# sourmash-bio/sourmash

Measured on AMD Instinct MI355X. Metric: Gbase/s sketched (k=31, scaled=1000), higher is better.
Workload: dtype u64; 1 GPU; C2: sketch synthetic random DNA resident in HBM as ASCII, per GPU 1000 records of 10000000 bases (10000000000 bases, 10000001000 bytes with their separators), k=31 scaled=1000 seed=42; one step = k-mer kernel + radix sort + unique; records_per_gpu=1000, record_len=10000000, bases_per_gpu=10000000000, bytes_per_gpu=10000001000, ksize=31, scaled=1000, unique_hashes_rank0=9998668, unique_hashes_job=9998668, collectives=none (the exchange runs with --full)

## Files before the change

include/sourmash_amd.h:

```cpp
#ifndef SOURMASH_AMD_H_INCLUDED
#define SOURMASH_AMD_H_INCLUDED

#include <stdarg.h>
#include <stdbool.h>
#include <stdint.h>
#include <stdlib.h>

#ifdef __cplusplus
extern "C" {
#endif


enum {
  HASH_FUNCTIONS_MURMUR64_DNA = 1,
  HASH_FUNCTIONS_MURMUR64_PROTEIN = 2,
  HASH_FUNCTIONS_MURMUR64_DAYHOFF = 3,
  HASH_FUNCTIONS_MURMUR64_HP = 4,
};
typedef uint32_t HashFunctions;

enum {
  SOURMASH_ERROR_CODE_NO_ERROR = 0,
  SOURMASH_ERROR_CODE_PANIC = 1,
  SOURMASH_ERROR_CODE_INTERNAL = 2,
// ... 166 lines not shown
SourmashHyperLogLog *hll_with_error_rate(double error_rate, uintptr_t ksize);

bool nodegraph_count(SourmashNodegraph *ptr, uint64_t h);
bool nodegraph_count_kmer(SourmashNodegraph *ptr, const char *kmer);
double nodegraph_expected_collisions(const SourmashNodegraph *ptr);
void nodegraph_free(SourmashNodegraph *ptr);
SourmashNodegraph *nodegraph_from_buffer(const char *ptr, uintptr_t insize);
SourmashNodegraph *nodegraph_from_path(const char *filename);
uintptr_t nodegraph_get(const SourmashNodegraph *ptr, uint64_t h);
uintptr_t nodegraph_get_kmer(const SourmashNodegraph *ptr, const char *kmer);
const uint64_t *nodegraph_hashsizes(const SourmashNodegraph *ptr, uintptr_t *size);
uintptr_t nodegraph_ksize(const SourmashNodegraph *ptr);
uintptr_t nodegraph_matches(const SourmashNodegraph *ptr, const SourmashKmerMinHash *mh_ptr);
SourmashNodegraph *nodegraph_new(void);
uintptr_t nodegraph_noccupied(const SourmashNodegraph *ptr);
uintptr_t nodegraph_ntables(const SourmashNodegraph *ptr);
void nodegraph_save(const SourmashNodegraph *ptr, const char *filename);
const uint8_t *nodegraph_to_buffer(const SourmashNodegraph *ptr, uint8_t compression, uintptr_t *size);
void nodegraph_update(SourmashNodegraph *ptr, const SourmashNodegraph *optr);
void nodegraph_update_mh(SourmashNodegraph *ptr, const SourmashKmerMinHash *optr);
SourmashNodegraph *nodegraph_with_tables(uintptr_t ksize, uintptr_t starting_size, uintptr_t n_tables);


int32_t smgpu_device_count(void);
bool smgpu_available(void);

void smgpu_minhash_add_buffer(SourmashKmerMinHash *ptr, const char *buf, uintptr_t len, bool force);

uint32_t smgpu_minhash_add_sequence_rc(SourmashKmerMinHash *ptr, const char *sequence, uintptr_t len, bool force);
void smgpu_minhash_flush(SourmashKmerMinHash *ptr);
uint64_t smgpu_minhash_pending_bytes(const SourmashKmerMinHash *ptr);
uint64_t smgpu_signature_add_file(SourmashSignature *ptr, const char *path, uint64_t *n_records);
SourmashSignature **smgpu_sketch_files(const char *const *paths, uintptr_t n, const SourmashComputeParameters *params,
                                       uint32_t n_threads, uint64_t *total_bases);
uint64_t smgpu_minhash_add_file(SourmashKmerMinHash *ptr, const char *path, uint64_t *n_records);
uint64_t smgpu_gunzip_files(const char *const *paths, uintptr_t n, uint8_t *out, uint64_t capacity, uint64_t *lens, double *stats);
void smgpu_sigload_counters(uint64_t *out);
void smgpu_gunzip_counters(uint64_t *out);

uint64_t smgpu_sketch_workspace_bytes(uint64_t out_capacity);
uint64_t smgpu_sketch_dna_raw(const uint8_t *d_seq, uint64_t len, uint32_t ksize, uint64_t seed, uint64_t max_hash,
                              uint64_t *d_out, uint64_t out_capacity, uint64_t *d_result, void *d_workspace,
                              uint64_t workspace_bytes, void *stream);
uint64_t smgpu_sketch_records_workspace_bytes(uint64_t pair_capacity, uint64_t n_records);
uint64_t smgpu_sketch_records_raw(const uint8_t *d_seq, uint64_t len, const uint64_t *d_starts, uint64_t n_records,
                                  uint32_t ksize, uint64_t seed, uint64_t max_hash, uint64_t *d_hashes, uint64_t *d_abunds,
                                  uint64_t capacity, uint64_t *d_offsets, uint64_t *d_result, void *d_workspace,
                                  uint64_t workspace_bytes, void *stream);
void smgpu_sketch_records_kernel_raw(const uint8_t *d_seq, uint64_t len, uint32_t ksize, uint64_t seed, uint64_t max_hash,
                                     uint64_t *d_hashes, uint64_t *d_positions, uint64_t capacity, uint64_t *d_count, void *stream);
SourmashSignature **smgpu_sketch_file_singleton(const char *path, const SourmashComputeParameters *params, uintptr_t *n);
void smgpu_sketch_dna_kernel_raw(const uint8_t *d_seq, uint64_t len, uint32_t ksize, uint64_t seed, uint64_t max_hash,
                                 uint64_t *d_out, uint64_t out_capacity, uint64_t *d_count, void *stream);
uint64_t smgpu_sort_unique_raw(uint64_t *d_keys, uint64_t n, uint64_t *d_out, uint64_t *d_n_out, void *d_workspace,
                               uint64_t workspace_bytes, void *stream);
uint64_t smgpu_sketch_residues_kernels_raw(const uint8_t *d_seq, uint64_t len, uint32_t k_aa, uint32_t hash_function, uint64_t seed,
                                           uint64_t max_hash, bool translate, uint8_t *d_aa, uint64_t aa_capacity, uint64_t *d_out,
                                           uint64_t out_capacity, uint64_t *d_count, void *stream);
void smgpu_synth_dna_raw(uint8_t *d_out, uint64_t start, uint64_t n, uint64_t seed, uint64_t record_len, void *stream);

void smgpu_compare_raw(const uint64_t *d_hashes, const uint64_t *d_offsets, uint32_t n, uint32_t row_lo,
                       uint32_t row_hi, uint32_t *d_common, double *d_jaccard, void *stream);
void smgpu_compare_blocks_raw(const uint64_t *d_hashes, const uint64_t *d_offsets, uint32_t n, uint32_t rb_first,
                              uint32_t rb_stride, uint32_t rb_count, uint32_t *d_common, void *stream);
void smgpu_symmetrize_raw(uint32_t *d_common, uint32_t n, void *stream);
void smgpu_jaccard_raw(const uint32_t *d_common, const uint64_t *d_offsets, uint32_t n, uint32_t row_lo,
                       uint32_t row_hi, double *d_jaccard, void *stream);
typedef struct SmgpuBitIndex SmgpuBitIndex;
SmgpuBitIndex *smgpu_bitindex_new(const uint64_t *d_hashes, const uint64_t *d_offsets, uint32_t n, void *stream);
SmgpuBitIndex *smgpu_bitindex_new_ex(const uint64_t *d_hashes, const uint64_t *d_offsets, uint32_t n, uint64_t total_hashes,
                                     uint32_t threshold, bool one_shot, void *stream);
void smgpu_bitindex_free(SmgpuBitIndex *ptr);
uint64_t smgpu_bitindex_universe(const SmgpuBitIndex *ptr);
uint32_t smgpu_bitindex_builder(const SmgpuBitIndex *ptr);
void smgpu_bitindex_stats(const SmgpuBitIndex *ptr, uint64_t *frequent_hashes, uint64_t *rare_pairs, uint32_t *threshold);
void smgpu_bitindex_compare_raw(const SmgpuBitIndex *ptr, uint32_t rb_first, uint32_t rb_stride, uint32_t rb_count,
                                uint32_t *d_common, void *stream);
void smgpu_bitindex_compare_upper_raw(const SmgpuBitIndex *ptr, uint32_t rb_first, uint32_t rb_stride, uint32_t rb_count,
                                      uint32_t *d_common, void *stream);
void smgpu_host_pow_f64(const double *x, const double *y, uintptr_t ny, double *out, uintptr_t n, uint32_t n_threads);
uintptr_t smgpu_first_invalid_dna_byte(const char *seq, uintptr_t len);
void smgpu_compare_all_pairs(const SourmashKmerMinHash *const *mhs, uintptr_t n, uint32_t *common_out,
                             double *jaccard_out);
void smgpu_compare_all_pairs_mixed(const SourmashKmerMinHash *const *mhs, uintptr_t n, const uint32_t *class_of,
                                   const uint64_t *class_max_hash, uintptr_t n_classes, uint32_t *common_out, uint64_t *sizes_out);
void smgpu_signatures_sketch_views(const SourmashSignature *const *sigs, uintptr_t n, const SourmashKmerMinHash **out_mhs,
                                   uint64_t *params);
void smgpu_minhashes_params(const SourmashKmerMinHash *const *mhs, uintptr_t n, uint64_t *params);
void *smgpu_host_alloc(uintptr_t bytes);
void smgpu_host_free(void *ptr);
void smgpu_xfer_stats(uint64_t *out5, bool reset);
void smgpu_xfer_roundtrip(const void *const *pieces, const uint64_t *lens, uintptr_t n, void *out, uint64_t out_bytes);
void smgpu_compare_num_all_pairs(const SourmashKmerMinHash *const *mhs, uintptr_t n, uint32_t *common_out, uint32_t *union_out,
                                 double *jaccard_out);
void smgpu_compare_angular_all_pairs(const SourmashKmerMinHash *const *mhs, uintptr_t n, double *sims_out, uint64_t *prod_out,
                                     uint64_t *sumsq_out);
void smgpu_host_angular_f64(const uint64_t *prod, const uint64_t *sumsq, uintptr_t n, double *out, uint32_t n_threads);
void smgpu_compare_num_raw(const uint64_t *d_hashes, const uint64_t *d_offsets, const uint32_t *d_nums, uint32_t n,
                           uint32_t *d_common, uint32_t *d_union, double *d_jaccard, void *stream);
void smgpu_compare_abund_raw(const uint64_t *d_hashes, const uint64_t *d_abunds, const uint64_t *d_offsets, uint32_t n, bool narrow,
                             uint32_t *d_common, uint64_t *d_prod, uint64_t *d_sumsq, void *stream);
void smgpu_compare_abund_raw_n(const uint64_t *d_hashes, const uint64_t *d_abunds, const uint64_t *d_offsets, uint32_t n,
                               uint64_t total_hashes, bool narrow, uint32_t *d_common, uint64_t *d_prod, uint64_t *d_sumsq, void *stream);

typedef struct SmgpuSketchSet SmgpuSketchSet;
typedef struct SmgpuCounter SmgpuCounter;
// ... 106 lines not shown
```

sourmash_amd/csrc/capi.cpp:

```cpp
#if defined(__SSE2__)
#include <emmintrin.h>
#endif
#include <hip/hip_runtime_api.h>
#include <stdio.h>
#include <string.h>
#include <chrono>
#include <cmath>
#include <fstream>
#include <memory>
#include <sstream>
#include <thread>
#include "../../include/sourmash_amd.h"
#include "collection.hpp"
#include <fcntl.h>
#include <sys/mman.h>
#include <sys/stat.h>
#include <unistd.h>
#include "device_ctx.hpp"
#include "hostxfer.hpp"
#include "pargz.hpp"
#include "ingest.hpp"
#include "sigload.hpp"
#include "murmur3.hpp"
#include "residues.hpp"
// ... 773 lines not shown
    return (uint64_t)out_capacity * 8 + sort_unique_temp_bytes(out_capacity) + 512;
}

uint64_t smgpu_sketch_dna_raw(const uint8_t* d_seq, uint64_t len, uint32_t ksize, uint64_t seed, uint64_t max_hash,
                              uint64_t* d_out, uint64_t cap, uint64_t* d_result, void* d_ws, uint64_t ws_bytes,
                              void* stream) {
    uint64_t ret = ~0ull;
    landing_void([&] {
        hipStream_t st = (hipStream_t)stream;
        if (ws_bytes < smgpu_sketch_workspace_bytes(cap)) throw err_internal("workspace too small (smgpu_sketch_workspace_bytes)");
        uint64_t* d_raw = (uint64_t*)d_ws;
        void* d_tmp = (char*)d_ws + ((cap * 8 + 255) / 256) * 256;
        const size_t tmp_bytes = (size_t)(ws_bytes - ((cap * 8 + 255) / 256) * 256);
        const uint64_t thr = max_hash ? max_hash : ~0ull;
        check_dna_ksize(ksize);
        hip_check(hipMemsetAsync(d_result, 0, 16, st), "memset");
        hip_check(sketch_dna_launch(d_seq, len, ksize, seed, thr, d_raw, (unsigned long long*)d_result, cap, st), "sketch_dna");
        unsigned long long kept = 0;
        hip_check(hipMemcpyAsync(&kept, d_result, 8, hipMemcpyDeviceToHost, st), "D2H");
        hip_check(hipStreamSynchronize(st), "sync");
        if (kept > cap)
            throw err_internal("output capacity too small: " + std::to_string(kept) + " kept hashes > capacity " + std::to_string(cap));
        int bits = 64;
        if (thr != ~0ull) { bits = 1; while (bits < 64 && (thr >> bits)) ++bits; }
        hip_check(sort_unique(d_raw, kept, d_out, nullptr, d_result + 1, d_tmp, tmp_bytes, bits, st), "sort_unique");
        unsigned long long nu = 0;
        hip_check(hipMemcpyAsync(&nu, d_result + 1, 8, hipMemcpyDeviceToHost, st), "D2H");
        hip_check(hipStreamSynchronize(st), "sync");
        ret = nu;
    });
    return ret;
}

uint64_t smgpu_sort_unique_raw(uint64_t* d_keys, uint64_t n, uint64_t* d_out, uint64_t* d_n_out, void* d_ws, uint64_t ws_bytes, void* stream) {
    uint64_t ret = ~0ull;
    landing_void([&] {
        hipStream_t st = (hipStream_t)stream;
        if (ws_bytes < sort_unique_temp_bytes(n)) throw err_internal("workspace too small (smgpu_sketch_workspace_bytes)");
        hip_check(sort_unique(d_keys, n, d_out, nullptr, d_n_out, d_ws, (size_t)ws_bytes, 64, st), "sort_unique");
        unsigned long long nu = 0;
        hip_check(hipMemcpyAsync(&nu, d_n_out, 8, hipMemcpyDeviceToHost, st), "D2H");
        hip_check(hipStreamSynchronize(st), "sync");
        ret = nu;
    });
    return ret;
}

void smgpu_sketch_dna_kernel_raw(const uint8_t* d_seq, uint64_t len, uint32_t ksize, uint64_t seed, uint64_t max_hash,
                                 uint64_t* d_out, uint64_t cap, uint64_t* d_count, void* stream) {
    landing_void([&] {
        check_dna_ksize(ksize);
        hip_check(sketch_dna_launch(d_seq, len, ksize, seed, max_hash ? max_hash : ~0ull, d_out,
                                    (unsigned long long*)d_count, cap, (hipStream_t)stream), "sketch_dna");
    });
}

uint64_t smgpu_sketch_residues_kernels_raw(const uint8_t* d_seq, uint64_t len, uint32_t k_aa, uint32_t hash_function, uint64_t seed,
                                           uint64_t max_hash, bool translate, uint8_t* d_aa, uint64_t aa_capacity, uint64_t* d_out,
                                           uint64_t cap, uint64_t* d_count, void* stream) {
    return landing<uint64_t>([&]() -> uint64_t {
        if (hash_function < HF_PROTEIN || hash_function > HF_HP) throw err_internal("hash_function must be protein, dayhoff or hp");
        const uint64_t n_aa = translate ? translated_bytes(len) : len;
        if (((n_aa + 7) & ~7ull) > aa_capacity) throw err_internal("d_aa is too small: " + std::to_string(n_aa) + " residues need " + std::to_string((n_aa + 7) & ~7ull) + " bytes");
        hipStream_t st = (hipStream_t)stream;
        if (translate) hip_check(translate_launch(d_seq, len, hash_function, d_aa, st), "translate");
        else hip_check(residues_launch(d_seq, len, hash_function, d_aa, st), "residues");
        hip_check(residue_windows_launch(d_aa, translate && len < 3 ? 0 : n_aa, k_aa, seed, max_hash ? max_hash : ~0ull, d_out, (unsigned long long*)d_count, cap,
                                         false, st), "residue windows");
        return n_aa;
    });
}

void smgpu_synth_dna_raw(uint8_t* d_out, uint64_t start, uint64_t n, uint64_t seed, uint64_t record_len, void* stream) {
    landing_void([&] { hip_check(synth_dna_launch(d_out, start, n, seed, record_len, (hipStream_t)stream), "synth_dna"); });
}

void smgpu_compare_raw(const uint64_t* d_hashes, const uint64_t* d_offsets, uint32_t n, uint32_t row_lo, uint32_t row_hi,
                       uint32_t* d_common, double* d_jaccard, void* stream) {
    landing_void([&] {
        if (!d_common) throw err_internal("d_common is required");
        hip_check(compare_counts_launch(d_hashes, d_offsets, n, row_lo, row_hi, d_common, (hipStream_t)stream), "compare");
        if (d_jaccard)
            hip_check(jaccard_from_counts_launch(d_common, d_offsets, n, row_lo, row_hi, d_jaccard, (hipStream_t)stream), "jaccard");
    });
}

void smgpu_compare_blocks_raw(const uint64_t* d_hashes, const uint64_t* d_offsets, uint32_t n, uint32_t rb_first,
                              uint32_t rb_stride, uint32_t rb_count, uint32_t* d_common, void* stream) {
    landing_void([&] {
        hip_check(compare_blocks_launch(d_hashes, d_offsets, n, rb_first, rb_stride, rb_count, d_common, (hipStream_t)stream),
                  "compare_blocks");
    });
}
void smgpu_symmetrize_raw(uint32_t* d_common, uint32_t n, void* stream) {
    landing_void([&] { hip_check(symmetrize_launch(d_common, n, (hipStream_t)stream), "symmetrize"); });
}
void smgpu_jaccard_raw(const uint32_t* d_common, const uint64_t* d_offsets, uint32_t n, uint32_t row_lo, uint32_t row_hi,
                       double* d_jaccard, void* stream) {
    landing_void([&] {
        hip_check(jaccard_from_counts_launch(d_common, d_offsets, n, row_lo, row_hi, d_jaccard, (hipStream_t)stream), "jaccard");
    });
}

struct BitIndex {
    uint32_t n = 0, words_per_row = 0;
    uint64_t universe = 0, total = 0;
// ... 2124 lines not shown
```

sourmash_amd/csrc/device_api.hpp:

```cpp
#pragma once
#include <hip/hip_runtime.h>
#include <stdint.h>
#include <stddef.h>

namespace smg {

hipError_t sketch_dna_launch(const uint8_t* d_seq, uint64_t len, uint32_t k, uint64_t seed, uint64_t thr,
                             uint64_t* d_out, unsigned long long* d_count, uint64_t cap, hipStream_t stream);
struct SketchMultiOut { uint64_t thr; uint64_t* out; unsigned long long* count; uint64_t cap; };
bool sketch_dna_multi_supported(const uint32_t* ks, int n);
hipError_t sketch_dna_multi_launch(const uint8_t* d_new, uint64_t n_new, const uint32_t* ks, int n, uint64_t seed, const SketchMultiOut* outs,
                                   hipStream_t stream);
hipError_t sketch_dna_words_launch(const uint8_t* d_seq, uint64_t len, uint32_t k, uint64_t seed, uint64_t thr, uint64_t* d_out,
                                   unsigned long long* d_count, uint64_t cap, bool dense, hipStream_t stream);
uint32_t sketch_dna_max_k();
hipError_t kmer_hashes_launch(const uint8_t* d_seq, uint64_t len, uint32_t k, uint64_t seed, uint64_t* d_out,
                              uint64_t n_kmers, hipStream_t stream);
hipError_t first_invalid_launch(const uint8_t* d_seq, uint64_t len, unsigned long long* d_first, hipStream_t stream);

hipError_t hll_dna_launch(const uint8_t* d_seq, uint64_t len, uint32_t k, uint32_t p, uint32_t* d_regs, hipStream_t stream);
hipError_t hll_hashes_launch(const uint64_t* d_hashes, uint64_t n, uint32_t p, uint32_t* d_regs, bool skip_zero, hipStream_t stream);
hipError_t hll_pack_launch(const uint32_t* d_regs, uint32_t n, uint8_t* d_out, hipStream_t stream);

struct NgTable { uint64_t size, magic, off; };
struct NgDev {
    const NgTable* tabs = nullptr;
    uint32_t n_tables = 0;
    uint32_t* words = nullptr;
    uint64_t n_words = 0;
    uint64_t t0_words = 0;
    unsigned long long* occ = nullptr;
};
hipError_t nodegraph_dna_launch(const uint8_t* d_seq, uint64_t len, uint32_t k, const NgDev& g, hipStream_t stream);
hipError_t nodegraph_hashes_launch(const uint64_t* d_hashes, uint64_t n, const NgDev& g, hipStream_t stream);
hipError_t nodegraph_matches_launch(const uint64_t* d_hashes, const uint64_t* d_offsets, uint64_t n_rows, const NgDev& g,
                                    uint64_t* d_out, hipStream_t stream);

hipError_t residues_launch(const uint8_t* d_seq, uint64_t len, uint32_t hash_function, uint8_t* d_aa, hipStream_t stream);
uint64_t translated_bytes(uint64_t len);
hipError_t translate_launch(const uint8_t* d_seq, uint64_t len, uint32_t hash_function, uint8_t* d_aa, hipStream_t stream);
hipError_t residue_windows_launch(const uint8_t* d_aa, uint64_t n, uint32_t k, uint64_t seed, uint64_t thr, uint64_t* d_out,
                                  unsigned long long* d_count, uint64_t cap, bool dense, hipStream_t stream);

size_t sort_unique_temp_bytes(uint64_t n);
struct TagSegment { uint64_t src, dst, n; };
hipError_t tag_gather_launch(const uint64_t* d_src, const TagSegment* d_segs, uint32_t n_segs, uint64_t* d_dst, int hbits, hipStream_t stream);
hipError_t sort_unique(uint64_t* d_keys, uint64_t n, uint64_t* d_out, uint64_t* d_counts, uint64_t* d_n_out,
                       void* d_temp, size_t temp_bytes, int bits, hipStream_t stream);

size_t sort_pairs_temp_bytes(uint64_t n);
hipError_t sort_pairs(const uint64_t* d_keys_in, uint64_t* d_keys_out, const uint64_t* d_vals_in, uint64_t* d_vals_out, uint64_t n,
                      int bits, void* d_temp, size_t temp_bytes, hipStream_t stream);
size_t rle_pairs_temp_bytes(uint64_t n);
hipError_t rle_pairs(const uint64_t* d_a, const uint64_t* d_b, uint64_t n, uint64_t* d_out_a, uint64_t* d_out_b, uint64_t* d_counts,
                     uint64_t* d_n_out, void* d_temp, size_t temp_bytes, hipStream_t stream);

hipError_t records_pairs_launch(const uint8_t* d_seq, uint64_t len, uint32_t k, uint64_t seed, uint64_t thr, uint64_t* d_hash,
                                uint64_t* d_pos, unsigned long long* d_count, uint64_t cap, hipStream_t stream);
hipError_t records_check_starts_launch(const uint64_t* d_starts, uint64_t n_records, uint64_t len, unsigned long long* d_bad,
                                       hipStream_t stream);
size_t records_csr_temp_bytes(uint64_t n_pairs);
// ... 58 lines not shown
```

sourmash_amd/csrc/kmer_core.hpp:

```cpp
#pragma once
#include "murmur3.hpp"
#include <utility>

namespace smg {

SMG_HD uint32_t perm_b32(uint32_t hi, uint32_t lo, uint32_t sel) {
#if defined(__HIP_DEVICE_COMPILE__)
    return __builtin_amdgcn_perm(hi, lo, sel);
#else
    const uint64_t v = ((uint64_t)hi << 32) | lo;
    uint32_t r = 0;
    for (int i = 0; i < 4; ++i) {
        const uint32_t s = (sel >> (8 * i)) & 0xff;
        uint32_t b;
        if (s < 8) b = (uint32_t)(v >> (8 * s)) & 0xff;
        else if (s == 0x0c) b = 0;
        else b = 0xff;
        r |= b << (8 * i);
    }
    return r;
#endif
}

SMG_HD uint32_t alignbyte_b32(uint32_t hi, uint32_t lo, uint32_t n) {
// ... 188 lines not shown
        }
    }
    static_assert(G::NBYTES <= 192 && K <= 128 && P <= 64, "window too long for the 192-bit validity mask");
    (
        [&] {
            const Mmh3Open open = PosOps<K, P, O>::template hash_open<PLAIN>(U, C, seed);
            if constexpr (EARLY) {
                if (!any_lane(early_may_keep(open, lim))) return;
            }
            const uint64_t h = mmh3_close<PLAIN>(open);
            bool ok = (h - 1) < thr;
            if (anybad != 0) {
                uint64_t lo, hi;
                if constexpr (O == 0) { lo = badlo; hi = badhi; }
                else { lo = (badlo >> O) | (badhi << (64 - O)); hi = (badhi >> O) | (badtop << (64 - O)); }
                const uint64_t mlo = K >= 64 ? ~0ull : ((1ull << K) - 1);
                const uint64_t mhi = K >= 128 ? ~0ull : K > 64 ? ((1ull << (K - 64)) - 1) : 0;
                if ((lo & mlo) | (hi & mhi)) ok = false;
            }
            if (ok) emit(O, h);
        }(),
        ...);
}

template <int K, int P, bool EARLY = true, bool PLAIN = false, class Emit>
SMG_HD void process_lane(const uint32_t* raw, uint64_t seed, uint64_t thr, Emit&& emit) {
    process_window<K, P, EARLY, PLAIN, false>(raw, nullptr, false, seed, thr, static_cast<Emit&&>(emit),
                                              std::make_integer_sequence<int, P>{});
}
template <int K, int P, bool EARLY = true, bool PLAIN = false, class Emit>
SMG_HD void process_lane_staged(const uint32_t* U, const uint32_t* C, bool dirty, uint64_t seed, uint64_t thr, Emit&& emit) {
    process_window<K, P, EARLY, PLAIN, true>(U, C, dirty, seed, thr, static_cast<Emit&&>(emit), std::make_integer_sequence<int, P>{});
}


template <int K, int P, int BLOCK, int R = 1>
struct TileGeom {
    using G = LaneGeom<K, P>;
    static constexpr int WINDOW = BLOCK * P;
    static constexpr int TILE = R * WINDOW;
    static constexpr int LANE_RD = ((G::NW + 3) / 4) * 4;
    static constexpr int chunks(int rounds) { return ((rounds * BLOCK - 1) * (P / 4) + LANE_RD + 3) / 4; }
    static constexpr int IN_DW = (R * BLOCK - 1) * (P / 4) + LANE_RD;
    static constexpr int IN_CHUNKS = chunks(R);
};

SMG_HD uint32_t sk_tile_rounds(uint64_t thr, uint32_t r_max, uint32_t window, uint32_t cap) {
    if (r_max <= 1) return 1;
    const uint64_t positions = (uint64_t)r_max * window;
    const uint64_t expected = (positions * (thr >> 32)) >> 32;
    return expected + 1 > cap / 4 ? 1u : r_max;
}

SMG_HD void load_chunk(const uint8_t* seq, uint64_t off, uint64_t len, uint32_t skip, uint32_t* w) {
    w[0] = w[1] = w[2] = w[3] = 0;
    if (off + 16 <= len) {
#if defined(__HIP_DEVICE_COMPILE__)
        const uint4 v = *reinterpret_cast<const uint4*>(seq + off);
        w[0] = v.x; w[1] = v.y; w[2] = v.z; w[3] = v.w;
#else
        for (int b = 0; b < 16; ++b) w[b >> 2] |= (uint32_t)seq[off + b] << (8 * (b & 3));
#endif
    } else if (off < len) {
        for (uint64_t b = off; b < len; ++b) w[(b - off) >> 2] |= (uint32_t)seq[b] << (8 * ((b - off) & 3));
    }
    if (off == 0 && skip) {
        for (uint32_t b = 0; b < skip; ++b) w[b >> 2] &= ~(0xffu << (8 * (b & 3)));
    }
}

SMG_HD uint32_t stage_chunk(uint32_t* w, uint32_t* c) {
    uint32_t anybad = 0;
#pragma unroll
    for (int j = 0; j < 4; ++j) {
        const uint32_t u = w[j] & 0xdfdfdfdfu;
        const uint32_t code = (u >> 1) & 0x03030303u;
        w[j] = u;
        c[j] = perm_b32(0u, LUT_COMP, code);
        anybad |= perm_b32(0u, LUT_SELF, code) ^ u;
    }
    return anybad;
}

SMG_HD void store_chunk(uint32_t* dst, const uint32_t* w) {
#if defined(__HIP_DEVICE_COMPILE__)
    *reinterpret_cast<uint4*>(dst) = make_uint4(w[0], w[1], w[2], w[3]);
#else
    dst[0] = w[0]; dst[1] = w[1]; dst[2] = w[2]; dst[3] = w[3];
#endif
}

template <int IN_CHUNKS, bool STAGED, int BLOCK>
SMG_HD void stage_tile(const uint8_t* seq, uint64_t base, uint64_t len, uint32_t skip, uint32_t* s_in, uint32_t* s_comp,
                       unsigned int* s_dirty, int n_chunks = IN_CHUNKS) {
#if defined(__HIP_DEVICE_COMPILE__)
    const int first = threadIdx.x, step = BLOCK;
#else
    const int first = 0, step = 1;
#endif
    for (int c = first; c < n_chunks; c += step) {
        uint32_t w[4];
        load_chunk(seq, base + (uint64_t)c * 16, len, skip, w);
        if constexpr (STAGED) {
            uint32_t cw[4];
            if (stage_chunk(w, cw)) *s_dirty = 1;
            store_chunk(&s_comp[c * 4], cw);
// ... 69 lines not shown
```

sourmash_amd/csrc/sketch.hip:

```cpp
#include <hip/hip_runtime.h>
#include <stdint.h>
#include <stdlib.h>
#include <utility>
#include "kmer_core.hpp"
#include "sketch_kernel.hpp"
#include "device_api.hpp"

namespace smg {

constexpr int GENERIC_MAX_K = 256;
constexpr int GENERIC_TILE = 4096;

__global__ __launch_bounds__(SK_BLOCK) void sketch_dna_generic_kernel(
    const uint8_t* __restrict__ seq, uint64_t len, uint32_t k, uint64_t seed, uint64_t thr,
    uint64_t* __restrict__ out, unsigned long long* __restrict__ out_count, uint64_t out_cap, uint64_t n_tiles,
    int dense) {
    __shared__ uint8_t s_in[GENERIC_TILE + GENERIC_MAX_K];
    for (uint64_t tile = blockIdx.x; tile < n_tiles; tile += gridDim.x) {
        const uint64_t base = tile * (uint64_t)GENERIC_TILE;
        __syncthreads();
        for (uint32_t i = threadIdx.x; i < GENERIC_TILE + k - 1; i += SK_BLOCK)
            s_in[i] = (base + i < len) ? seq[base + i] : 0;
        __syncthreads();
        for (uint32_t p = threadIdx.x; p < GENERIC_TILE; p += SK_BLOCK) {
            uint8_t fwd[GENERIC_MAX_K], rev[GENERIC_MAX_K];
            bool ok = true;
            for (uint32_t j = 0; j < k; ++j) {
                const uint8_t u = s_in[p + j] & 0xdf;
                uint8_t c;
                switch (u) {
                case 'A': c = 'T'; break;
                case 'C': c = 'G'; break;
                case 'G': c = 'C'; break;
                case 'T': c = 'A'; break;
                default: c = 0; ok = false;
                }
                fwd[j] = u;
                rev[k - 1 - j] = c;
            }
            if (!ok) continue;
            bool use_rev = false;
            for (uint32_t j = 0; j < k; ++j) {
                if (fwd[j] != rev[j]) { use_rev = rev[j] < fwd[j]; break; }
            }
            const uint64_t h = mmh3_h1_bytes(use_rev ? rev : fwd, k, seed);
            if ((h - 1) < thr) {
                if (dense) {
                    if (base + p < out_cap) out[base + p] = h;
                } else {
                    const unsigned long long g = atomicAdd(out_count, 1ull);
                    if (g < out_cap) out[g] = h;
                }
            }
        }
    }
}

__global__ __launch_bounds__(SK_BLOCK) void first_invalid_kernel(const uint8_t* __restrict__ seq, uint64_t len,
                                                                unsigned long long* __restrict__ first) {
    unsigned long long best = ~0ull;
    for (uint64_t i = (uint64_t)blockIdx.x * SK_BLOCK + threadIdx.x; i < len; i += (uint64_t)gridDim.x * SK_BLOCK) {
        const uint8_t u = seq[i] & 0xdf;
        if (!(u == 'A' || u == 'C' || u == 'G' || u == 'T')) { best = i; break; }
    }
    if (best != ~0ull) atomicMin(first, best);
}

constexpr int FAST_MAX_K = SK_FAST_MAX_K;
SMG_KMER_PART(SketchLaunch<false>, 0)
SMG_KMER_PART(SketchLaunch<false>, 1)
SMG_KMER_PART(SketchLaunch<false>, 2)
SMG_KMER_PART(SketchLaunch<false>, 3)

static hipError_t sketch_any(const uint8_t* d_seq, uint64_t len, uint32_t k, uint64_t seed, uint64_t thr,
                             uint64_t* d_out, unsigned long long* d_count, uint64_t cap, bool dense,
                             hipStream_t stream) {
    if (len < k || k == 0) return hipSuccess;
    static const bool generic_only = [] { const char* e = getenv("SMG_SKETCH_GENERIC"); return e && *e == '1'; }();
    constexpr uint32_t words_from = (uint32_t)FAST_MAX_K + 1u;
    if (k >= words_from && !generic_only) return sketch_dna_words_launch(d_seq, len, k, seed, thr, d_out, d_count, cap, dense, stream);
    if (!dense && k <= (uint32_t)FAST_MAX_K && !generic_only)
        return launcher<SketchLaunch<false>>(k)(d_seq, len, seed, thr, d_out, d_count, cap, stream);
    if (dense && k <= (uint32_t)FAST_MAX_K && !generic_only)
        return launcher<SketchLaunch<true>>(k)(d_seq, len, seed, thr, d_out, d_count, cap, stream);
    if (!generic_only || k > (uint32_t)GENERIC_MAX_K) return sketch_dna_words_launch(d_seq, len, k, seed, thr, d_out, d_count, cap, dense, stream);
    const uint64_t n_tiles = (len + GENERIC_TILE - 1) / GENERIC_TILE;
    hipLaunchKernelGGL(sketch_dna_generic_kernel, dim3(sk_grid(n_tiles)), dim3(SK_BLOCK), 0, stream, d_seq, len, k, seed, thr,
                       d_out, d_count, cap, n_tiles, dense ? 1 : 0);
    return hipGetLastError();
}

hipError_t sketch_dna_launch(const uint8_t* d_seq, uint64_t len, uint32_t k, uint64_t seed, uint64_t thr,
                             uint64_t* d_out, unsigned long long* d_count, uint64_t cap, hipStream_t stream) {
    return sketch_any(d_seq, len, k, seed, thr, d_out, d_count, cap, false, stream);
}

hipError_t kmer_hashes_launch(const uint8_t* d_seq, uint64_t len, uint32_t k, uint64_t seed, uint64_t* d_out,
                              uint64_t n_kmers, hipStream_t stream) {
    return sketch_any(d_seq, len, k, seed, ~0ull, d_out, nullptr, n_kmers, true, stream);
}

hipError_t first_invalid_launch(const uint8_t* d_seq, uint64_t len, unsigned long long* d_first, hipStream_t stream) {
    if (len == 0) return hipSuccess;
    const uint64_t nb = (len + SK_BLOCK - 1) / SK_BLOCK;
    const unsigned grid = (unsigned)(nb < 2048 ? nb : 2048);
    hipLaunchKernelGGL(first_invalid_kernel, dim3(grid), dim3(SK_BLOCK), 0, stream, d_seq, len, d_first);
    return hipGetLastError();
}

}
```

sourmash_amd/csrc/sketch_kernel.hpp:

```cpp
#pragma once
#include <hip/hip_runtime.h>
#include <stdint.h>
#include <utility>
#include "kmer_core.hpp"
#include "tile_launch.hpp"

namespace smg {

constexpr int SK_BLOCK = 256;
constexpr int SK_FAST_MAX_K = 88;
constexpr int SK_OUT_CAP = 2048;

constexpr bool sk_plain_mul(int k, bool dense) {
    if (dense) return k == 1 || k == 5 || k == 8 || k == 25 || k == 28 || k == 81 || k == 82 || k == 84;
    return k == 50 || k == 51;
}
constexpr bool sk_staged(int k) { return k > 11 && k != 18 && k != 20 && k != 30; }
#ifndef SMG_SK_R_MAX
#define SMG_SK_R_MAX 3
#endif
constexpr int SK_R_MAX = SMG_SK_R_MAX;
static_assert(SK_R_MAX >= 1 && SK_R_MAX <= 3, "four rounds do not fit four workgroups per CU");
constexpr bool sk_one_round(int k) { return k <= 17; }
constexpr int sk_rounds_max(int k, bool dense) { return !dense && sk_staged(k) && !sk_one_round(k) ? SK_R_MAX : 1; }
constexpr int sk_out_cap(int r_max) { return r_max >= 3 ? SK_OUT_CAP / 2 : SK_OUT_CAP; }
#ifdef SMG_SK_GRID_PER_CU
constexpr unsigned sk_grid_per_cu(int) { return SMG_SK_GRID_PER_CU; }
#else
constexpr unsigned sk_grid_per_cu(int r_max) { return r_max > 1 ? 32 : 8; }
#endif

template <int K, int P, bool DENSE>
__global__ __launch_bounds__(SK_BLOCK) void sketch_dna_kernel(
    const uint8_t* __restrict__ seq, uint64_t len, uint64_t seed, uint64_t thr,
    uint64_t* __restrict__ out, unsigned long long* __restrict__ out_count, uint64_t out_cap,
    uint64_t n_tiles, uint32_t skip, uint32_t rounds) {
    constexpr int R_MAX = sk_rounds_max(K, DENSE), OUT_CAP = sk_out_cap(R_MAX);
    using T = TileGeom<K, P, SK_BLOCK, R_MAX>;
    constexpr int WINDOW = T::WINDOW, LANE_RD = T::LANE_RD, IN_CHUNKS = T::IN_CHUNKS;
    constexpr bool STAGED = !DENSE && sk_staged(K);
    static_assert(R_MAX == 1 || STAGED, "only the staged form walks several rounds");
    const uint32_t n_rounds = R_MAX > 1 ? rounds : 1u;

    __shared__ __attribute__((aligned(16))) uint32_t s_in[IN_CHUNKS * 4];
    __shared__ __attribute__((aligned(16))) uint32_t s_comp[STAGED ? IN_CHUNKS * 4 : 4];
    __shared__ unsigned int s_dirty;
    __shared__ uint64_t s_out[OUT_CAP];
    __shared__ unsigned int s_cnt;
    __shared__ unsigned long long s_base;
    const LdsSink<OUT_CAP, SK_BLOCK> sink{{s_out}, &s_cnt, &s_base, {out}, out_count, out_cap};

    const int tid = threadIdx.x;
    if (tid == 0) s_cnt = 0;

    for (uint64_t tile = blockIdx.x; tile < n_tiles; tile += gridDim.x) {
        const uint64_t base = tile * ((uint64_t)n_rounds * WINDOW);
        if constexpr (STAGED) {
            if (tid == 0) s_dirty = 0;
        }
        __syncthreads();
        if constexpr (STAGED) {
            if constexpr (R_MAX > 1) stage_tile<IN_CHUNKS, true, SK_BLOCK>(seq, base, len, skip, s_in, s_comp, &s_dirty, T::chunks((int)n_rounds));
            else stage_tile<IN_CHUNKS, true, SK_BLOCK>(seq, base, len, skip, s_in, s_comp, &s_dirty);
        } else {
            for (int c = tid; c < IN_CHUNKS; c += SK_BLOCK) {
                const uint64_t off = base + (uint64_t)c * 16;
                uint4 v = make_uint4(0, 0, 0, 0);
                if (off + 16 <= len) {
                    v = *reinterpret_cast<const uint4*>(seq + off);
                } else if (off < len) {
                    uint32_t w[4] = {0, 0, 0, 0};
                    for (uint64_t b = off; b < len; ++b) w[(b - off) >> 2] |= (uint32_t)seq[b] << (8 * ((b - off) & 3));
                    v = make_uint4(w[0], w[1], w[2], w[3]);
                }
                if (off == 0 && skip) {
                    uint32_t w[4] = {v.x, v.y, v.z, v.w};
                    for (uint32_t b = 0; b < skip; ++b) w[b >> 2] &= ~(0xffu << (8 * (b & 3)));
                    v = make_uint4(w[0], w[1], w[2], w[3]);
                }
                *reinterpret_cast<uint4*>(&s_in[c * 4]) = v;
            }
        }
        __syncthreads();
        uint32_t raw[LANE_RD];
        if constexpr (R_MAX == 1) read_window<LANE_RD, P>(s_in, tid, raw);
        auto emit = [&](int o, uint64_t h) {
            if constexpr (DENSE) {
                const uint64_t pos = base + (uint64_t)tid * P + (uint64_t)o - skip;
                if (pos < out_cap) out[pos] = h;
            } else {
                sink.append(h);
            }
        };
        if constexpr (STAGED) {
            static_assert(!STAGED || P == 16, "the staged form reads whole 16-byte groups");
            uint32_t comp[LANE_RD];
            if constexpr (R_MAX == 1) {
                read_window<LANE_RD, P>(s_comp, tid, comp);
                const bool dirty = __builtin_amdgcn_readfirstlane(s_dirty) != 0;
                process_lane_staged<K, P, true, sk_plain_mul(K, false)>(raw, comp, dirty, seed, thr, emit);
            } else {
                const bool dirty = __builtin_amdgcn_readfirstlane(s_dirty) != 0;
#pragma unroll 1
                for (uint32_t r = 0; r < n_rounds; ++r) {
                    read_window<LANE_RD, P>(s_in, tid + (int)r * SK_BLOCK, raw);
                    read_window<LANE_RD, P>(s_comp, tid + (int)r * SK_BLOCK, comp);
                    process_lane_staged<K, P, true, sk_plain_mul(K, false)>(raw, comp, dirty, seed, thr, emit);
                }
            }
        } else {
            process_lane<K, P, !DENSE, sk_plain_mul(K, DENSE)>(raw, seed, thr, emit);
        }
        if constexpr (DENSE) continue;
        __syncthreads();
        sink.flush(OUT_CAP / 2);
    }
    if constexpr (DENSE) return;
    __syncthreads();
    sink.flush(1);
}

typedef hipError_t (*sketch_launch_fn)(const uint8_t*, uint64_t, uint64_t, uint64_t, uint64_t*, unsigned long long*, uint64_t, hipStream_t);
template <bool DENSE>
struct SketchLaunch {
    using fn = sketch_launch_fn;
    static constexpr int KMAX = SK_FAST_MAX_K;
    template <int K>
    static hipError_t launch(const uint8_t* d_seq, uint64_t len, uint64_t seed, uint64_t thr, uint64_t* d_out,
                             unsigned long long* d_count, uint64_t cap, hipStream_t stream) {
        constexpr uint32_t WINDOW = (uint32_t)SK_BLOCK * 16, R_MAX = (uint32_t)sk_rounds_max(K, DENSE);
        const uint32_t rounds = sk_tile_rounds(thr, R_MAX, WINDOW, (uint32_t)sk_out_cap((int)R_MAX));
        const TileSpan t = align_to_tiles(d_seq, len, (uint64_t)rounds * WINDOW);
        if (t.n_tiles == 0) return hipSuccess;
        hipLaunchKernelGGL((sketch_dna_kernel<K, 16, DENSE>), dim3(sk_grid(t.n_tiles, sk_grid_per_cu((int)R_MAX))), dim3(SK_BLOCK), 0, stream,
                           t.seq, t.len, seed, thr, d_out, d_count, cap, t.n_tiles, t.skip, rounds);
        return hipGetLastError();
    }
};

}
```

sourmash_amd/device.py:

```python
import ctypes as C

from ._lowlevel import lib
from .minhash import _get_max_hash_for_scaled
from .exceptions import SourmashError, exceptions_by_code
from .utils import decode_str, rustcall


def _torch():
    import torch
    if not torch.cuda.is_available():
        raise RuntimeError("sourmash_amd.device needs a HIP device (no CPU fallback)")
    return torch


def _ptr(t):
    return C.c_void_p(t.data_ptr())


def _stream(torch):
    return C.c_void_p(torch.cuda.current_stream().cuda_stream)


def _u64(torch, n, device):
    return torch.empty(int(n), dtype=torch.int64, device=device)
# ... 52 lines not shown
        torch = self.torch
        assert seq.dtype == torch.uint8 and seq.is_cuda and seq.is_contiguous()
        n = seq.numel()
        self._reserve(self.capacity_for(n))
        for attempt in range(2):
            lib.sourmash_err_clear()
            got = lib.smgpu_sketch_dna_raw(_ptr(seq), n, self.ksize, self.seed, self.max_hash, _ptr(self.out),
                                           self.cap, _ptr(self.result), _ptr(self.ws), self.ws.numel(),
                                           _stream(torch))
            code = lib.sourmash_err_get_last_code()
            if code == 0:
                return self.out[:got]
            message = decode_str(lib.sourmash_err_get_last_message())
            kept = int(self.result[0].item())
            if attempt == 0 and kept > self.cap:
                self._reserve(kept + 1024)
                continue
            raise exceptions_by_code.get(code, SourmashError)(message)

    def sketch_records(self, seq, starts, *, abund=False):
        torch = self.torch
        assert seq.dtype == torch.uint8 and seq.is_cuda and seq.is_contiguous()
        assert starts.dtype == torch.int64 and starts.is_cuda and starts.is_contiguous()
        if starts.numel() < 1:
            raise ValueError("record starts: n_records + 1 offsets are needed")
        n, n_records = seq.numel(), starts.numel() - 1
        expect = n / max(self.scaled, 1)
        cap = max(1, min(n, int(expect * 2 + 16 * (expect + 1) ** 0.5) + 4096))
        result = torch.zeros(4, dtype=torch.int64, device=seq.device)
        offsets = _u64(torch, n_records + 1, seq.device)
        for attempt in range(2):
            hashes = _u64(torch, cap, seq.device)
            abunds = _u64(torch, cap, seq.device) if abund else None
            ws = torch.empty(int(lib.smgpu_sketch_records_workspace_bytes(cap, n_records)), dtype=torch.uint8, device=seq.device)
            lib.sourmash_err_clear()
            got = lib.smgpu_sketch_records_raw(_ptr(seq), n, _ptr(starts), n_records, self.ksize, self.seed, self.max_hash,
                                               _ptr(hashes), _ptr(abunds) if abund else None, cap, _ptr(offsets), _ptr(result),
                                               _ptr(ws), ws.numel(), _stream(torch))
            code = lib.sourmash_err_get_last_code()
            if code == 0:
                return (hashes[:got], offsets, abunds[:got]) if abund else (hashes[:got], offsets)
            message = decode_str(lib.sourmash_err_get_last_message())
            kept = int(result[0].item())
            if attempt == 0 and kept > cap:
                cap = kept
                continue
            raise _records_error(code, message)

    def records_kernel_only(self, seq, out_hashes, out_positions, count):
        torch = self.torch
        rustcall(lib.smgpu_sketch_records_kernel_raw, _ptr(seq), seq.numel(), self.ksize, self.seed, self.max_hash,
                 _ptr(out_hashes), _ptr(out_positions), min(out_hashes.numel(), out_positions.numel()), _ptr(count), _stream(torch))

    def kernel_only(self, seq, out, count):
        torch = self.torch
        rustcall(lib.smgpu_sketch_dna_kernel_raw, _ptr(seq), seq.numel(), self.ksize, self.seed, self.max_hash,
                 _ptr(out), out.numel(), _ptr(count), _stream(torch))


def sort_unique(keys):
    torch = _torch()
    assert keys.dtype == torch.int64 and keys.is_cuda and keys.is_contiguous()
    n = keys.numel()
    out = _u64(torch, max(n, 1), keys.device)
    if n == 0:
        return out[:0]
    ws = torch.empty(int(lib.smgpu_sketch_workspace_bytes(n)), dtype=torch.uint8, device=keys.device)
    n_out = torch.zeros(1, dtype=torch.int64, device=keys.device)
    m = rustcall(lib.smgpu_sort_unique_raw, _ptr(keys), n, _ptr(out), _ptr(n_out), _ptr(ws), ws.numel(), _stream(torch))
    return out[:m]


def pack_csr(sketches, device="cuda"):
    import numpy as np
    torch = _torch()
    offsets = np.zeros(len(sketches) + 1, dtype=np.int64)
    for i, s in enumerate(sketches):
        offsets[i + 1] = offsets[i] + len(s)
    flat = np.concatenate([np.asarray(s, dtype=np.uint64) for s in sketches]) if len(sketches) and offsets[-1] \
        else np.zeros(0, dtype=np.uint64)
    hashes = torch.from_numpy(flat.view(np.int64).copy()).to(device)
    if hashes.numel() == 0:
        hashes = torch.zeros(2, dtype=torch.int64, device=device)
    return hashes, torch.from_numpy(offsets).to(device)


class BitIndex:

    def __init__(self, ptr, n):
        self._ptr, self.n = ptr, n

    @classmethod
    def build(cls, hashes, offsets, threshold=None, one_shot=False):
        torch = _torch()
        n = offsets.numel() - 1
        ptr = rustcall(lib.smgpu_bitindex_new_ex, _ptr(hashes), _ptr(offsets), n, 0, int(threshold or 0), bool(one_shot),
                       _stream(torch))
        return cls(ptr, n) if ptr else None

    @property
    def universe(self):
        return lib.smgpu_bitindex_universe(self._ptr)

    @property
    def builder(self):
        return {1: "dictionary", 2: "sort"}.get(int(lib.smgpu_bitindex_builder(self._ptr)), "?")

    @property
    def stats(self):
        f, r, t = C.c_uint64(), C.c_uint64(), C.c_uint32()
# ... 45 lines not shown
```

Baseline: 360.7 Gbase/s.

## Hand out sketch tiles dynamically via atomic ticket counter on a resident grid

```diff
diff --git a/include/sourmash_amd.h b/include/sourmash_amd.h
--- a/include/sourmash_amd.h
+++ b/include/sourmash_amd.h
@@ -242,6 +242,8 @@
 SourmashSignature **smgpu_sketch_file_singleton(const char *path, const SourmashComputeParameters *params, uintptr_t *n);
 void smgpu_sketch_dna_kernel_raw(const uint8_t *d_seq, uint64_t len, uint32_t ksize, uint64_t seed, uint64_t max_hash,
                                  uint64_t *d_out, uint64_t out_capacity, uint64_t *d_count, void *stream);
+void smgpu_sketch_dna_kernel_grid_raw(const uint8_t *d_seq, uint64_t len, uint32_t ksize, uint64_t seed, uint64_t max_hash,
+                                      uint64_t *d_out, uint64_t out_capacity, uint64_t *d_count, uint32_t grid, void *stream);
 uint64_t smgpu_sort_unique_raw(uint64_t *d_keys, uint64_t n, uint64_t *d_out, uint64_t *d_n_out, void *d_workspace,
                                uint64_t workspace_bytes, void *stream);
 uint64_t smgpu_sketch_residues_kernels_raw(const uint8_t *d_seq, uint64_t len, uint32_t k_aa, uint32_t hash_function, uint64_t seed,
diff --git a/sourmash_amd/csrc/capi.cpp b/sourmash_amd/csrc/capi.cpp
--- a/sourmash_amd/csrc/capi.cpp
+++ b/sourmash_amd/csrc/capi.cpp
@@ -849,6 +849,15 @@
         check_dna_ksize(ksize);
         hip_check(sketch_dna_launch(d_seq, len, ksize, seed, max_hash ? max_hash : ~0ull, d_out,
                                     (unsigned long long*)d_count, cap, (hipStream_t)stream), "sketch_dna");
+    });
+}
+void smgpu_sketch_dna_kernel_grid_raw(const uint8_t* d_seq, uint64_t len, uint32_t ksize, uint64_t seed, uint64_t max_hash,
+                                      uint64_t* d_out, uint64_t cap, uint64_t* d_count, uint32_t grid, void* stream) {
+    landing_void([&] {
+        check_dna_ksize(ksize);
+        if (grid > (1u << 20)) throw err_internal("grid: at most 1048576 workgroups");
+        hip_check(sketch_dna_launch_grid(d_seq, len, ksize, seed, max_hash ? max_hash : ~0ull, d_out,
+                                         (unsigned long long*)d_count, cap, grid, (hipStream_t)stream), "sketch_dna");
     });
 }
 
diff --git a/sourmash_amd/csrc/device_api.hpp b/sourmash_amd/csrc/device_api.hpp
--- a/sourmash_amd/csrc/device_api.hpp
+++ b/sourmash_amd/csrc/device_api.hpp
@@ -7,6 +7,8 @@
 
 hipError_t sketch_dna_launch(const uint8_t* d_seq, uint64_t len, uint32_t k, uint64_t seed, uint64_t thr,
                              uint64_t* d_out, unsigned long long* d_count, uint64_t cap, hipStream_t stream);
+hipError_t sketch_dna_launch_grid(const uint8_t* d_seq, uint64_t len, uint32_t k, uint64_t seed, uint64_t thr,
+                                  uint64_t* d_out, unsigned long long* d_count, uint64_t cap, uint32_t grid, hipStream_t stream);
 struct SketchMultiOut { uint64_t thr; uint64_t* out; unsigned long long* count; uint64_t cap; };
 bool sketch_dna_multi_supported(const uint32_t* ks, int n);
 hipError_t sketch_dna_multi_launch(const uint8_t* d_new, uint64_t n_new, const uint32_t* ks, int n, uint64_t seed, const SketchMultiOut* outs,
diff --git a/sourmash_amd/csrc/kmer_core.hpp b/sourmash_amd/csrc/kmer_core.hpp
--- a/sourmash_amd/csrc/kmer_core.hpp
+++ b/sourmash_amd/csrc/kmer_core.hpp
@@ -264,6 +264,10 @@
     return expected + 1 > cap / 4 ? 1u : r_max;
 }
 
+SMG_HD uint64_t tile_first(uint32_t workgroup) { return workgroup; }
+SMG_HD uint64_t tile_from_ticket(uint32_t grid, uint64_t ticket) { return (uint64_t)grid + ticket; }
+SMG_HD bool tile_end(uint64_t tile, uint64_t n_tiles) { return tile >= n_tiles; }
+
 SMG_HD void load_chunk(const uint8_t* seq, uint64_t off, uint64_t len, uint32_t skip, uint32_t* w) {
     w[0] = w[1] = w[2] = w[3] = 0;
     if (off + 16 <= len) {
diff --git a/sourmash_amd/csrc/sketch.hip b/sourmash_amd/csrc/sketch.hip
--- a/sourmash_amd/csrc/sketch.hip
+++ b/sourmash_amd/csrc/sketch.hip
@@ -74,15 +74,15 @@
 
 static hipError_t sketch_any(const uint8_t* d_seq, uint64_t len, uint32_t k, uint64_t seed, uint64_t thr,
                              uint64_t* d_out, unsigned long long* d_count, uint64_t cap, bool dense,
-                             hipStream_t stream) {
+                             hipStream_t stream, uint32_t grid = 0) {
     if (len < k || k == 0) return hipSuccess;
     static const bool generic_only = [] { const char* e = getenv("SMG_SKETCH_GENERIC"); return e && *e == '1'; }();
     constexpr uint32_t words_from = (uint32_t)FAST_MAX_K + 1u;
     if (k >= words_from && !generic_only) return sketch_dna_words_launch(d_seq, len, k, seed, thr, d_out, d_count, cap, dense, stream);
     if (!dense && k <= (uint32_t)FAST_MAX_K && !generic_only)
-        return launcher<SketchLaunch<false>>(k)(d_seq, len, seed, thr, d_out, d_count, cap, stream);
+        return launcher<SketchLaunch<false>>(k)(d_seq, len, seed, thr, d_out, d_count, cap, grid, stream);
     if (dense && k <= (uint32_t)FAST_MAX_K && !generic_only)
-        return launcher<SketchLaunch<true>>(k)(d_seq, len, seed, thr, d_out, d_count, cap, stream);
+        return launcher<SketchLaunch<true>>(k)(d_seq, len, seed, thr, d_out, d_count, cap, 0, stream);
     if (!generic_only || k > (uint32_t)GENERIC_MAX_K) return sketch_dna_words_launch(d_seq, len, k, seed, thr, d_out, d_count, cap, dense, stream);
     const uint64_t n_tiles = (len + GENERIC_TILE - 1) / GENERIC_TILE;
     hipLaunchKernelGGL(sketch_dna_generic_kernel, dim3(sk_grid(n_tiles)), dim3(SK_BLOCK), 0, stream, d_seq, len, k, seed, thr,
@@ -93,6 +93,11 @@
 hipError_t sketch_dna_launch(const uint8_t* d_seq, uint64_t len, uint32_t k, uint64_t seed, uint64_t thr,
                              uint64_t* d_out, unsigned long long* d_count, uint64_t cap, hipStream_t stream) {
     return sketch_any(d_seq, len, k, seed, thr, d_out, d_count, cap, false, stream);
+}
+
+hipError_t sketch_dna_launch_grid(const uint8_t* d_seq, uint64_t len, uint32_t k, uint64_t seed, uint64_t thr,
+                                  uint64_t* d_out, unsigned long long* d_count, uint64_t cap, uint32_t grid, hipStream_t stream) {
+    return sketch_any(d_seq, len, k, seed, thr, d_out, d_count, cap, false, stream, grid);
 }
 
 hipError_t kmer_hashes_launch(const uint8_t* d_seq, uint64_t len, uint32_t k, uint64_t seed, uint64_t* d_out,
diff --git a/sourmash_amd/csrc/sketch_kernel.hpp b/sourmash_amd/csrc/sketch_kernel.hpp
--- a/sourmash_amd/csrc/sketch_kernel.hpp
+++ b/sourmash_amd/csrc/sketch_kernel.hpp
@@ -4,6 +4,7 @@
 #include <utility>
 #include "kmer_core.hpp"
 #include "tile_launch.hpp"
+#include "arena.hpp"
 
 namespace smg {
 
@@ -24,17 +25,22 @@
 constexpr bool sk_one_round(int k) { return k <= 17; }
 constexpr int sk_rounds_max(int k, bool dense) { return !dense && sk_staged(k) && !sk_one_round(k) ? SK_R_MAX : 1; }
 constexpr int sk_out_cap(int r_max) { return r_max >= 3 ? SK_OUT_CAP / 2 : SK_OUT_CAP; }
+#ifdef SMG_SK_STATIC_WALK
+constexpr bool sk_handout(int) { return false; }
+#else
+constexpr bool sk_handout(int) { return true; }
+#endif
 #ifdef SMG_SK_GRID_PER_CU
-constexpr unsigned sk_grid_per_cu(int) { return SMG_SK_GRID_PER_CU; }
+constexpr unsigned sk_grid_per_cu(int, bool) { return SMG_SK_GRID_PER_CU; }
 #else
-constexpr unsigned sk_grid_per_cu(int r_max) { return r_max > 1 ? 32 : 8; }
+constexpr unsigned sk_grid_per_cu(int r_max, bool handout) { return handout ? 0 : r_max > 1 ? 32 : 8; }
 #endif
 
 template <int K, int P, bool DENSE>
 __global__ __launch_bounds__(SK_BLOCK) void sketch_dna_kernel(
     const uint8_t* __restrict__ seq, uint64_t len, uint64_t seed, uint64_t thr,
     uint64_t* __restrict__ out, unsigned long long* __restrict__ out_count, uint64_t out_cap,
-    uint64_t n_tiles, uint32_t skip, uint32_t rounds) {
+    uint64_t n_tiles, uint32_t skip, uint32_t rounds, unsigned long long* __restrict__ tile_counter) {
     constexpr int R_MAX = sk_rounds_max(K, DENSE), OUT_CAP = sk_out_cap(R_MAX);
     using T = TileGeom<K, P, SK_BLOCK, R_MAX>;
     constexpr int WINDOW = T::WINDOW, LANE_RD = T::LANE_RD, IN_CHUNKS = T::IN_CHUNKS;
@@ -48,12 +54,15 @@
     __shared__ uint64_t s_out[OUT_CAP];
     __shared__ unsigned int s_cnt;
     __shared__ unsigned long long s_base;
+    __shared__ unsigned long long s_next;
+    const bool handout = !DENSE && sk_handout(K) && tile_counter != nullptr;
     const LdsSink<OUT_CAP, SK_BLOCK> sink{{s_out}, &s_cnt, &s_base, {out}, out_count, out_cap};
 
     const int tid = threadIdx.x;
     if (tid == 0) s_cnt = 0;
 
-    for (uint64_t tile = blockIdx.x; tile < n_tiles; tile += gridDim.x) {
+    uint64_t tile = tile_first(blockIdx.x);
+    while (!tile_end(tile, n_tiles)) {
         const uint64_t base = tile * ((uint64_t)n_rounds * WINDOW);
         if constexpr (STAGED) {
             if (tid == 0) s_dirty = 0;
@@ -82,6 +91,9 @@
             }
         }
         __syncthreads();
+        if constexpr (!DENSE && sk_handout(K)) {
+            if (handout && tid == 0) s_next = tile_from_ticket(gridDim.x, atomicAdd(tile_counter, 1ull));
+        }
         uint32_t raw[LANE_RD];
         if constexpr (R_MAX == 1) read_window<LANE_RD, P>(s_in, tid, raw);
         auto emit = [&](int o, uint64_t h) {
@@ -111,8 +123,15 @@
         } else {
             process_lane<K, P, !DENSE, sk_plain_mul(K, DENSE)>(raw, seed, thr, emit);
         }
-        if constexpr (DENSE) continue;
+        if constexpr (DENSE) { tile += gridDim.x; continue; }
         __syncthreads();
+        if (handout) {
+            const unsigned long long next = s_next;
+            tile = ((uint64_t)(uint32_t)__builtin_amdgcn_readfirstlane((int)(uint32_t)(next >> 32)) << 32) |
+                   (uint32_t)__builtin_amdgcn_readfirstlane((int)(uint32_t)next);
+        } else {
+            tile += gridDim.x;
+        }
         sink.flush(OUT_CAP / 2);
     }
     if constexpr (DENSE) return;
@@ -120,20 +139,52 @@
     sink.flush(1);
 }
 
-typedef hipError_t (*sketch_launch_fn)(const uint8_t*, uint64_t, uint64_t, uint64_t, uint64_t*, unsigned long long*, uint64_t, hipStream_t);
+typedef hipError_t (*sketch_launch_fn)(const uint8_t*, uint64_t, uint64_t, uint64_t, uint64_t*, unsigned long long*, uint64_t, uint32_t, hipStream_t);
+template <int K, bool DENSE>
+unsigned sk_resident_grid() {
+    static const unsigned resident = [] {
+        int per_cu = 0, dev = 0, cus = 0;
+        if (hipOccupancyMaxActiveBlocksPerMultiprocessor(&per_cu, (const void*)sketch_dna_kernel<K, 16, DENSE>, SK_BLOCK, 0) != hipSuccess ||
+            hipGetDevice(&dev) != hipSuccess || hipDeviceGetAttribute(&cus, hipDeviceAttributeMultiprocessorCount, dev) != hipSuccess ||
+            per_cu < 1 || cus < 1) {
+            (void)hipGetLastError();
+            return 2048u;
+        }
+        return (unsigned)per_cu * (unsigned)cus;
+    }();
+    return resident;
+}
 template <bool DENSE>
 struct SketchLaunch {
     using fn = sketch_launch_fn;
     static constexpr int KMAX = SK_FAST_MAX_K;
     template <int K>
     static hipError_t launch(const uint8_t* d_seq, uint64_t len, uint64_t seed, uint64_t thr, uint64_t* d_out,
-                             unsigned long long* d_count, uint64_t cap, hipStream_t stream) {
+                             unsigned long long* d_count, uint64_t cap, uint32_t grid, hipStream_t stream) {
         constexpr uint32_t WINDOW = (uint32_t)SK_BLOCK * 16, R_MAX = (uint32_t)sk_rounds_max(K, DENSE);
         const uint32_t rounds = sk_tile_rounds(thr, R_MAX, WINDOW, (uint32_t)sk_out_cap((int)R_MAX));
         const TileSpan t = align_to_tiles(d_seq, len, (uint64_t)rounds * WINDOW);
         if (t.n_tiles == 0) return hipSuccess;
-        hipLaunchKernelGGL((sketch_dna_kernel<K, 16, DENSE>), dim3(sk_grid(t.n_tiles, sk_grid_per_cu((int)R_MAX))), dim3(SK_BLOCK), 0, stream,
-                           t.seq, t.len, seed, thr, d_out, d_count, cap, t.n_tiles, t.skip, rounds);
+        constexpr unsigned per_cu = sk_grid_per_cu((int)R_MAX, !DENSE && sk_handout(K));
+        unsigned g;
+        if (grid && !DENSE) {
+            g = grid;
+        } else if constexpr (per_cu == 0) {
+            const unsigned resident = sk_resident_grid<K, DENSE>();
+            g = (unsigned)(t.n_tiles < resident ? t.n_tiles : resident);
+        } else {
+            g = sk_grid(t.n_tiles, per_cu);
+        }
+        ArenaBuf counter;
+        if constexpr (!DENSE && sk_handout(K)) {
+            if (t.n_tiles > g) {
+                hipError_t e = counter.get(8, stream);
+                if (e == hipSuccess) e = hipMemsetAsync(counter.p, 0, 8, stream);
+                if (e != hipSuccess) return e;
+            }
+        }
+        hipLaunchKernelGGL((sketch_dna_kernel<K, 16, DENSE>), dim3(g), dim3(SK_BLOCK), 0, stream,
+                           t.seq, t.len, seed, thr, d_out, d_count, cap, t.n_tiles, t.skip, rounds, counter.as<unsigned long long>());
         return hipGetLastError();
     }
 };
diff --git a/sourmash_amd/device.py b/sourmash_amd/device.py
--- a/sourmash_amd/device.py
+++ b/sourmash_amd/device.py
@@ -128,10 +128,10 @@
         rustcall(lib.smgpu_sketch_records_kernel_raw, _ptr(seq), seq.numel(), self.ksize, self.seed, self.max_hash,
                  _ptr(out_hashes), _ptr(out_positions), min(out_hashes.numel(), out_positions.numel()), _ptr(count), _stream(torch))
 
-    def kernel_only(self, seq, out, count):
-        torch = self.torch
-        rustcall(lib.smgpu_sketch_dna_kernel_raw, _ptr(seq), seq.numel(), self.ksize, self.seed, self.max_hash,
-                 _ptr(out), out.numel(), _ptr(count), _stream(torch))
+    def kernel_only(self, seq, out, count, grid=0):
+        torch = self.torch
+        rustcall(lib.smgpu_sketch_dna_kernel_grid_raw, _ptr(seq), seq.numel(), self.ksize, self.seed, self.max_hash,
+                 _ptr(out), out.numel(), _ptr(count), int(grid), _stream(torch))
 
 
 def sort_unique(keys):
```

After: 370.6 Gbase/s, median of 6. 2.7% higher.
